# nicolapiccinelli/libmpc

Measured on AMD Instinct MI355X. Metric: MPC solves/sec (whole node) + p50 solve latency, quadrotor LMPC N=20 batch=4096, higher is better.
Workload: dtype f64; 1 GPU; quadrotor_ex.cpp LMPC nx=12 nu=4 ny=12 ph=ch=20, batch 4096 per GPU, SplitMix64 x0/u0/yref (SURVEY 8d), maximum_iteration=250; parallelism=single GPU, rccl_ranks=0, streams=1

## Files before the change

### libmpc_amd/csrc/lmpc_fast.hip

```cpp
#include "lmpc_kernel_common.hpp"
#include <cstddef>
#include <cstdlib>
#include <utility>

namespace mpcx {

namespace {

#ifndef MPCX_FAST_PF_MAXCAP
#define MPCX_FAST_PF_MAXCAP 12
#endif
#ifndef MPCX_FAST_RB
#define MPCX_FAST_RB 4
#endif
#ifndef MPCX_FAST_PF
#define MPCX_FAST_PF 4
#endif
#ifndef MPCX_FAST_PF_ALL
#define MPCX_FAST_PF_ALL 6
#endif
#ifndef MPCX_FAST_NBUF
#define MPCX_FAST_NBUF 3
#endif
#ifndef MPCX_FAST_RB_DEEP
#define MPCX_FAST_RB_DEEP 2
#endif
#ifndef MPCX_FAST_DEEP_CHUNKS
#define MPCX_FAST_DEEP_CHUNKS 4
#endif
#ifndef MPCX_FAST_XBAR_CLASSES
#define MPCX_FAST_XBAR_CLASSES 0
#endif
#ifndef MPCX_FAST_LDSMULT_CLASSES
#define MPCX_FAST_LDSMULT_CLASSES 0x30
#endif
#ifndef MPCX_FAST_XBAR_CHUNKS
#define MPCX_FAST_XBAR_CHUNKS 4
#endif
#ifndef MPCX_FAST_XBAR_CHUNK
#define MPCX_FAST_XBAR_CHUNK 0x333442400ull
#endif
constexpr int fast_xbar_chunk(int cap) { return (int)((MPCX_FAST_XBAR_CHUNK >> (4 * (cap / 2))) & 15) > 0 ? (int)((MPCX_FAST_XBAR_CHUNK >> (4 * (cap / 2))) & 15) : 1; }
constexpr bool fast_class_bit(unsigned mask, int cap, int chunks) { return chunks <= MPCX_FAST_XBAR_CHUNKS && ((mask >> (cap / 2)) & 1u) != 0; }
#ifndef MPCX_FAST_STAGE
#define MPCX_FAST_STAGE() __builtin_amdgcn_sched_barrier(0)
#endif
constexpr int kFastCap = 16;
#ifndef MPCX_FAST_ADD_THETA_LATE
#define MPCX_FAST_ADD_THETA_LATE 0.02
#endif
#ifndef MPCX_FAST_SAFE_AFTER
#define MPCX_FAST_SAFE_AFTER 12
#endif

template <int CTRL>
__device__ __forceinline__ double dpp_mov_d(double v)
{
    const int lo = __builtin_amdgcn_mov_dpp(__double2loint(v), CTRL, 0xF, 0xF, true);
    const int hi = __builtin_amdgcn_mov_dpp(__double2hiint(v), CTRL, 0xF, 0xF, true);
    return __hiloint2double(hi, lo);
}
__device__ __forceinline__ double wave_max_dpp(double v)
{
    v = fmax(v, dpp_mov_d<0xB1>(v));
    v = fmax(v, dpp_mov_d<0x4E>(v));
    v = fmax(v, dpp_mov_d<0x141>(v));
    v = fmax(v, dpp_mov_d<0x140>(v));
    v = fmax(v, dpp_mov_d<0x142>(v));
    v = fmax(v, dpp_mov_d<0x143>(v));
    return readlane_d(v, 63);
}

#ifdef MPCX_PROFILE_ROUNDS
#define MPCX_LAP(k) do { const long long now_ = (long long)__builtin_readcyclecounter(); pacc[k] += now_ - plast; plast = now_; } while (0)
#define MPCX_LAP_WAIT(k) do { __builtin_amdgcn_s_waitcnt(0); MPCX_LAP(k); } while (0)
#define MPCX_PROF_ARGS , long long (&pacc)[6], long long &plast
#define MPCX_PROF_PASS , pacc, plast
#else
#define MPCX_LAP(k) do {} while (0)
#define MPCX_LAP_WAIT(k) do {} while (0)
#define MPCX_PROF_ARGS
#define MPCX_PROF_PASS
#endif

template <int CAP, int NLO, int CPZ, int CPG, bool XB = false, bool XL = false>
__device__ __forceinline__ int ws_solve_reg(const gdp gY, const int ldy, const int ldz, const int na, const int lane_in,
                                            const int *wsidx, const double *wsb, const double *t0s, double *lam,
                                            const unsigned (&offz)[CPZ], const unsigned (&offg)[CPG],
                                            double (&wv)[2 * CPZ], double (&gw)[2 * CPG], double &lmax MPCX_PROF_ARGS)
{
    constexpr bool DEEP = CPZ + CPG <= MPCX_FAST_DEEP_CHUNKS;
    constexpr int PF = CAP > MPCX_FAST_PF_MAXCAP ? 0 : (CAP <= (DEEP ? MPCX_FAST_PF_ALL : MPCX_FAST_PF) ? CAP : MPCX_FAST_PF);
    int lane = lane_in;
    asm volatile("" : "+v"(lane));
    const bool real = lane < na;
    const int li = real ? lane : 0;
    const int qi = wsidx[li];
    int qc[CAP];
#pragma unroll
    for (int c = 0; c < CAP; ++c) qc[c] = __builtin_amdgcn_readfirstlane(wsidx[(c < NLO || c < na) ? c : 0]);
    double Sr[CAP];
    const unsigned rowoff = (unsigned)(qi * ldy) * 8u;
    const char MPCX_GAS *const gYb = reinterpret_cast<const char MPCX_GAS *>(gY);
    auto y_at = [&](unsigned off) { return *reinterpret_cast<gdp>(gYb + off); };
    auto row_ld2 = [&](int q, unsigned off) { return *reinterpret_cast<const d2 MPCX_GAS *>(gYb + (unsigned)(q * ldy) * 8u + off); };
#pragma unroll
    for (int c = 0; c < CAP; ++c) Sr[c] = y_at(rowoff + (unsigned)qc[c] * 8u);
    const double dg = y_at(rowoff + (unsigned)qi * 8u);
    d2 pz[PF > 0 ? PF : 1][CPZ], pg[PF > 0 ? PF : 1][CPG];
#pragma unroll
    for (int u = 0; u < PF; ++u) {
#pragma unroll
        for (int c = 0; c < CPZ; ++c) pz[u][c] = row_ld2(qc[u], offz[c]);
#pragma unroll
        for (int c = 0; c < CPG; ++c) pg[u][c] = row_ld2(qc[u], offg[c]);
    }
    double y = real ? t0s[qi < ldz ? qi : qi - ldz + 128 * CPZ] - wsb[li] : 0.0;
    MPCX_LAP_WAIT(1);
    if (!real) {
#pragma unroll
        for (int c = 0; c < CAP; ++c) Sr[c] = 0.0;
    }
#pragma unroll
    for (int c = NLO; c < CAP; ++c) if (c >= na) Sr[c] = lane == c ? 1.0 : 0.0;
    const double pthr = 1e-11 * (real ? dg : 1.0);
    double mydinv = 1.0;
    unsigned long long dep = 0ull;
    auto gj_step = [&]<int K>() {
        dep |= __ballot(!(Sr[K] > pthr)) & (1ull << K);
        const double rinv = pivot_rcp(readlane_d(Sr[K], K));
        if constexpr (XB) {
            constexpr int NE = CAP - K, XCH = fast_xbar_chunk(CAP), NC = (NE + XCH - 1) / XCH;
            double pv[2][XCH];
            auto request = [&](const int c) {
#pragma unroll
                for (int u = 0; u < XCH; ++u) {
                    const int j = K + 1 + c * XCH + u;
                    if (j <= CAP) pv[c & 1][u] = swizzle_bcast_d<K>(j < CAP ? Sr[j < CAP ? j : 0] : y);
                }
            };
            request(0);
            if (lane == K) mydinv = rinv;
            asm volatile("" : "+v"(mydinv));
            const double m = Sr[K] * rinv;
#pragma unroll
            for (int c = 0; c < NC; ++c) {
                if (c + 1 < NC) request(c + 1);
                if (lane != K) {
#pragma unroll
                    for (int u = 0; u < XCH; ++u) {
                        const int j = K + 1 + c * XCH + u;
                        if (j < CAP) Sr[j] = fma(-m, pv[c & 1][u], Sr[j]);
                        else if (j == CAP) y = fma(-m, pv[c & 1][u], y);
                    }
                }
            }
        } else {
            double pj[CAP];
#pragma unroll
            for (int j = K + 1; j < CAP; ++j) pj[j] = readlane_d(Sr[j], K);
            const double py = readlane_d(y, K);
            if (lane == K) mydinv = rinv;
            else {
                const double m = Sr[K] * rinv;
#pragma unroll
                for (int j = K + 1; j < CAP; ++j) Sr[j] = fma(-m, pj[j], Sr[j]);
                y = fma(-m, py, y);
            }
        }
    };
    [&]<int... Ks>(std::integer_sequence<int, Ks...>) { (gj_step.template operator()<Ks>(), ...); }(std::make_integer_sequence<int, CAP>{});
    MPCX_LAP(2);
    if (dep != 0ull) return (int)__builtin_ctzll(dep);
    y *= mydinv;
    if (XL ? lane < CAP : real) lam[lane] = y;
    auto lam_pair = [&](const int a, double (&l2)[2]) {
        const double2 v = *reinterpret_cast<const double2 *>(lam + a);
        l2[0] = v.x; l2[1] = v.y;
    };
    constexpr int NLP = XL && PF > 0 ? PF / 2 : 1;
    double lamp[NLP][2];
    if constexpr (XL) {
        static_assert(CAP % 2 == 0 && PF % 2 == 0 && kFastCap % 2 == 0, "multipliers are read back in pairs");
        wave_sync();
#pragma unroll
        for (int p = 0; p < PF / 2; ++p) lam_pair(2 * p, lamp[p]);
    }
#pragma unroll
    for (int c = 0; c < CPZ; ++c) {
        const double2 v = *reinterpret_cast<const double2 *>(t0s + 128 * c + 2 * lane);
        wv[2 * c] = v.x; wv[2 * c + 1] = v.y;
    }
#pragma unroll
    for (int c = 0; c < CPG; ++c) {
        const double2 v = *reinterpret_cast<const double2 *>(t0s + 128 * CPZ + 128 * c + 2 * lane);
        gw[2 * c] = v.x; gw[2 * c + 1] = v.y;
// ... 211 lines not shown
    }
    const int solver_status = infeasible ? -3 : (fixed_violation ? -2 : 1);

    double w[NZS], f[NZS];
    const double qnan = __builtin_nan("");
#pragma unroll
    for (int c = 0; c < CPZ; ++c) {
        const double2 vf = *reinterpret_cast<const double2 *>(fs + 128 * c + 2 * lane);
        f[2 * c] = vf.x; f[2 * c + 1] = vf.y;
    }
#pragma unroll
    for (int s = 0; s < NZS; ++s) w[s] = infeasible ? qnan : ((128 * (s >> 1) + 2 * lane + (s & 1) < nz) ? wv[s] : 0.0);
    double *stage = fs;
    double cost;
    bool cost_pending = false;
    wave_sync();
#pragma unroll
    for (int c = 0; c < CPZ; ++c) *reinterpret_cast<double2 *>(stage + 128 * c + 2 * lane) = make_double2(w[2 * c], w[2 * c + 1]);
    wave_sync();
    if (infeasible) {
        cost = 1e30;
    } else if (!M.cost_direct) {
        double j = 0;
#pragma unroll
        for (int s = 0; s < NZS; ++s) j = fma(f[s], w[s], j);
        if (lane < na_last) j = fma(-lam[lane], wsb[lane], j);
        cost = 0.5 * wave_sum(j) + c0;
    } else if (!FUSED && Bt.n_models <= 0) {
#pragma unroll
        for (int c = 0; c < CPZ; ++c) {
            const int e = 128 * c + 2 * lane;
            if (e < ldz) st2(ws + ldz + e, w[2 * c], w[2 * c + 1]);
        }
        cost = 0.0;
        cost_pending = true;
    } else {
        double hw[NZS];
#pragma unroll
        for (int s = 0; s < NZS; ++s) hw[s] = 0;
        matvec_acc<CPZ>(GP(H), ldz, ldz, nz, stage, hw, lane);
        double j = 0;
#pragma unroll
        for (int s = 0; s < NZS; ++s) j += w[s] * (0.5 * hw[s] + f[s]);
        cost = wave_sum(j) + c0;
    }
#pragma unroll
    for (int s = 0; s < NZS; ++s) {
        const int e = 128 * (s >> 1) + 2 * lane + (s & 1);
        if (e < nu) { if (outs) outs[8 + e] = w[s]; else glw(Bt.cmd)[(size_t)b * nu + e] = w[s]; }
    }
    if (outs) {
        if (lane == 0) {
            outs[0] = cost; outs[1] = solver_status == 1 ? 0 : (solver_status == -2 ? 1 : 2); outs[2] = solver_status;
            outs[3] = solver_status == -3 ? 0 : 1; outs[4] = 0; outs[5] = rounds_total; outs[6] = infeasible ? 0 : na_last; outs[7] = 2.0;
        }
    } else if (lane == 0) {
        if (Bt.cost && !cost_pending) glw(Bt.cost)[b] = cost;
        if (Bt.solver_status) glw(Bt.solver_status)[b] = solver_status;
        if (Bt.status) glw(Bt.status)[b] = solver_status == 1 ? 0 : (solver_status == -2 ? 1 : 2);
        if (Bt.is_feasible) glw(Bt.is_feasible)[b] = solver_status == -3 ? 0 : 1;
        if (Bt.iterations) glw(Bt.iterations)[b] = 0;
        if (Bt.polish_rounds) glw(Bt.polish_rounds)[b] = rounds_total;
        if (Bt.active_count) glw(Bt.active_count)[b] = infeasible ? 0 : na_last;
    }

    if (Bt.active_lower && Bt.active_upper) {
        wave_sync();
        unsigned *bl = reinterpret_cast<unsigned *>(t0s);
        unsigned *bu = bl + M.active_words;
        for (int wd = lane; wd < 2 * M.active_words; wd += 64) bl[wd] = 0u;
        wave_sync();
        if (!infeasible) {
#pragma unroll
            for (int s = 0; s < NZS; ++s) {
                const int e = 128 * (s >> 1) + 2 * lane + (s & 1);
                if (e >= nz || actb[s] == 0) continue;
                const double l = lam[posb[s]];
                if (!(fabs(l) > dtol_last)) continue;
                const int side = l < 0 ? -1 : 1;
                const double lo = lws[e], hi = uws[e];
                for (int p = GP(boxrow_ptr)[e]; p < GP(boxrow_ptr)[e + 1]; ++p) {
                    const int rr = GP(boxrow_ref)[p];
                    if (side < 0 && GP(boxrow_lo)[p] == lo) atomicOr(&bl[rr >> 5], 1u << (rr & 31));
                    if (side > 0 && GP(boxrow_hi)[p] == hi) atomicOr(&bu[rr >> 5], 1u << (rr & 31));
                }
            }
#pragma unroll
            for (int s = 0; s < NGS; ++s) {
                const int r = 128 * (s >> 1) + 2 * lane + (s & 1);
                if (r >= mg || actg[s] == 0) continue;
                const double l = lam[posg[s]];
                if (!(fabs(l) > dtol_last)) continue;
                const int rr = GP(g_refrow)[r];
                if (l < 0) atomicOr(&bl[rr >> 5], 1u << (rr & 31));
                else atomicOr(&bu[rr >> 5], 1u << (rr & 31));
            }
        }
        wave_sync();
        for (int wd = lane; wd < M.active_words; wd += 64) {
            glw(Bt.active_lower)[(size_t)b * M.active_words + wd] = bl[wd];
            glw(Bt.active_upper)[(size_t)b * M.active_words + wd] = bu[wd];
        }
        wave_sync();
    }

    if (Bt.seq_state || Bt.seq_input || Bt.seq_output) {
        wave_sync();
        const gdp gA = GP(A), gB = GP(B), gC = GP(C), gBd = GP(Bd), gDd = GP(Dd), gdm = gl(Bt.dmeas ? Bt.dmeas : M.dmeas_s);
        const gip gblk = GP(blk);
        auto dm = [&](int k, int dd) -> double { return ref_at(gdm, Bt.dmeas_bs, Bt.dmeas_ks, b, k, dd); };
        double *xs0 = scratch, *xs1 = scratch + nx;
        if (lane < nx) xs0[lane] = infeasible ? qnan : gl(Bt.x0)[(size_t)b * nx + lane];
        wave_sync();
        for (int i = 0; i <= ph; ++i) {
            const double *xc = (i & 1) ? xs1 : xs0;
            double *xn = (i & 1) ? xs0 : xs1;
            const int k = i > 0 ? i - 1 : 0;
            if (Bt.seq_state && lane < nx) glw(Bt.seq_state)[((size_t)b * (ph + 1) + i) * nx + lane] = xc[lane];
            if (Bt.seq_input && lane < nu) {
                const int ii = (i + 1 <= ph) ? i + 1 : ph;
                glw(Bt.seq_input)[((size_t)b * (ph + 1) + i) * nu + lane] = stage[gblk[ii] * nu + lane];
            }
            if (Bt.seq_output && lane < ny) {
                double yv = 0;
                for (int c = 0; c < nx; ++c) yv = fma(gC[lane + c * ny], xc[c], yv);
                if (M.has_dist) for (int dd = 0; dd < ndu; ++dd) yv = fma(gDd[lane + dd * ny], dm(k, dd), yv);
                glw(Bt.seq_output)[((size_t)b * (ph + 1) + i) * ny + lane] = yv;
            }
            if (i < ph && lane < nx) {
                double s = 0;
                for (int c = 0; c < nx; ++c) s = fma(gA[lane + c * nx], xc[c], s);
                for (int c = 0; c < nu; ++c) s = fma(gB[lane + c * nx], stage[gblk[i + 1] * nu + c], s);
                if (M.has_dist) for (int dd = 0; dd < ndu; ++dd) s = fma(gBd[lane + dd * nx], dm(i, dd), s);
                xn[lane] = s;
            }
            wave_sync();
        }
    }
    wave_sync();
    if (lane == 0 && !outs) ws[ldz + ldy + 2 * ldg + 1] = cost_pending ? 3.0 : 2.0;
    stamp(ts3);
    if (Bt.dbg_cycles && lane == 0)
    {
        long long *o = Bt.dbg_cycles + (size_t)b * 8;
#ifdef MPCX_PROFILE_ROUNDS
        o[0] = ts1 - ts0; o[1] = ts2 - ts1;
        for (int k = 0; k < 6; ++k) o[2 + k] = pacc[k];
#else
        o[0] = ts0; o[1] = ts1; o[2] = ts2; o[3] = ts3;
#endif
    }
}

template <int CPZ, int CPG, int SRC = 0>
__device__ __forceinline__ void solve_fast(const LmpcDev &M, const LmpcBatchDev &Bt, const int b, const int lane,
                           double *slice, const double *lwuw, gdw ws, const double *mf_lds = nullptr, double *outs = nullptr, const int eqbits = 0)
{
    constexpr int NZS = 2 * CPZ, NGS = 2 * CPG, ZP = 128 * CPZ, GPD = 128 * CPG;
    const int nz = M.nz, mg = M.mg, ldz = M.ldz, ldg = M.ldg, ldy = M.ldy;
    const gdp gY = GP(Y);
    double *t0s = slice, *gt0s = t0s + ZP, *lgs = gt0s + GPD, *ugs = lgs + GPD, *fs = ugs + GPD, *tail = fs + ZP;
    double *lam = tail + 2, *wsb = lam + (kFastCap + 2);
    int *wsidx = reinterpret_cast<int *>(wsb + (kFastCap + 2));
    double *scratch = wsb + (kFastCap + 2) + (kFastCap + 2) / 2 + 1;
    const double *lws = lwuw, *uws = lwuw + ZP;
    const double INF = __builtin_huge_val();

    long long ts0 = 0, ts1 = 0, ts2 = 0;
#ifdef MPCX_PROFILE_ROUNDS
    long long pacc[6] = {0, 0, 0, 0, 0, 0}, plast = 0;
#endif
    auto stamp = [&](long long &t) { if (Bt.dbg_cycles) t = (long long)__builtin_readcyclecounter(); };
    stamp(ts0);

    int offz[CPZ], offg[CPG];
#pragma unroll
    for (int c = 0; c < CPZ; ++c) { const int e = 128 * c + 2 * lane; offz[c] = e < ldz ? e : 0; }
#pragma unroll
    for (int c = 0; c < CPG; ++c) { const int r = 128 * c + 2 * lane; offg[c] = ldz + (r < ldg ? r : 0); }
    unsigned boffz[CPZ], boffg[CPG];
#pragma unroll
    for (int c = 0; c < CPZ; ++c) boffz[c] = (unsigned)offz[c] * 8u;
#pragma unroll
    for (int c = 0; c < CPG; ++c) boffg[c] = (unsigned)offg[c] * 8u;

    if constexpr (SRC != 2) fast_init_pads<CPZ, CPG>(slice, ldz, ldg, lane);
    if constexpr (SRC == 2) {
    } else if constexpr (SRC == 1) {
        RecPtrs rp{fs, t0s, gt0s, lgs, ugs, tail};
        fused_record(M, Bt, b, lane, scratch, rp, mf_lds);
    } else {
#pragma unroll
        for (int c = 0; c < CPZ; ++c) {
            const int e = 128 * c + 2 * lane;
            if (e < ldz) {
                const d2 vf = ld2(ws + e), vt = ld2(ws + ldz + e);
                *reinterpret_cast<double2 *>(fs + e) = make_double2(vf.x, vf.y);
                *reinterpret_cast<double2 *>(t0s + e) = make_double2(vt.x, vt.y);
            }
        }
#pragma unroll
        for (int c = 0; c < CPG; ++c) {
            const int r = 128 * c + 2 * lane;
            if (r < ldg) {
                const d2 vt = ld2(ws + 2 * ldz + r), vl = ld2(ws + ldz + ldy + r), vu = ld2(ws + ldz + ldy + ldg + r);
                *reinterpret_cast<double2 *>(gt0s + r) = make_double2(vt.x, vt.y);
                *reinterpret_cast<double2 *>(lgs + r) = make_double2(vl.x, vl.y);
                *reinterpret_cast<double2 *>(ugs + r) = make_double2(vu.x, vu.y);
            }
        }
        if (lane == 0) { const d2 t = ld2(ws + ldz + ldy + 2 * ldg); *reinterpret_cast<double2 *>(tail) = make_double2(t.x, t.y); }
        wave_sync();
    }
    const double flag0 = tail[1];
    const bool fixed_violation = flag0 == 1.0;
    const bool infeasible = fixed_violation && M.strict_infeasible;

    int actb[NZS], actg[NGS];
    const double ptol = 1e-8;
    auto viol = [&](double v, double lo, double hi) {
        const double lo_wide = fma(-ptol, fmax(1.0, fabs(lo)), lo), hi_scale = fmax(1.0, fabs(hi));
        return fmax(fmax(lo_wide - v, fma(-ptol, hi_scale, v - hi)), 0.0);
    };
    auto wrong_signed = [](double lm, int act) {
        const int in = -(act & 1);
        const int hi = (__double2hiint(lm) ^ (int)((unsigned)(act + 1) << 30)) & in;
        return __hiloint2double(hi, __double2loint(lm) & in);
    };
    {
        double vb[NZS], vg[NGS], vinit = 0.0;
        bool lowb[NZS], lowg[NGS];
#pragma unroll
        for (int c = 0; c < CPZ; ++c) {
            const int e = 128 * c + 2 * lane;
            const double2 l = *reinterpret_cast<const double2 *>(lws + e), u = *reinterpret_cast<const double2 *>(uws + e);
            const double2 t = *reinterpret_cast<const double2 *>(t0s + e);
            vb[2 * c] = viol(t.x, l.x, u.x); vb[2 * c + 1] = viol(t.y, l.y, u.y);
            lowb[2 * c] = t.x < l.x; lowb[2 * c + 1] = t.y < l.y;
            actb[2 * c] = l.x == u.x ? 2 : 0; actb[2 * c + 1] = l.y == u.y ? 2 : 0;
            vinit = fmax(vinit, fmax(vb[2 * c], vb[2 * c + 1]));
        }
#pragma unroll
        for (int c = 0; c < CPG; ++c) {
            const int r = 128 * c + 2 * lane;
            const double2 l = *reinterpret_cast<const double2 *>(lgs + r), u = *reinterpret_cast<const double2 *>(ugs + r);
            const double2 t = *reinterpret_cast<const double2 *>(gt0s + r);
            vg[2 * c] = viol(t.x, l.x, u.x); vg[2 * c + 1] = viol(t.y, l.y, u.y);
            lowg[2 * c] = t.x < l.x; lowg[2 * c + 1] = t.y < l.y;
            if constexpr (SRC == 2) {
                actg[2 * c] = ((eqbits >> (2 * c)) & 1) ? 2 : 0; actg[2 * c + 1] = ((eqbits >> (2 * c + 1)) & 1) ? 2 : 0;
            } else {
                const d2 l0 = ld2(GP(lg0) + (offg[c] - ldz)), u0 = ld2(GP(ug0) + (offg[c] - ldz));
                const bool ok = r < ldg;
                actg[2 * c] = (ok && l0.x == u0.x) ? 2 : 0; actg[2 * c + 1] = (ok && l0.y == u0.y) ? 2 : 0;
            }
            vinit = fmax(vinit, fmax(vg[2 * c], vg[2 * c + 1]));
        }
        const double thr0 = MPCX_INIT_THETA * wave_max_dpp(vinit);
#pragma unroll
        for (int s = 0; s < NZS; ++s) actb[s] = (actb[s] == 0 && vb[s] > 0.0 && vb[s] >= thr0) ? (lowb[s] ? -1 : 1) : actb[s];
#pragma unroll
        for (int s = 0; s < NGS; ++s) actg[s] = (actg[s] == 0 && vg[s] > 0.0 && vg[s] >= thr0) ? (lowg[s] ? -1 : 1) : actg[s];
    }
    stamp(ts1);

    if (Bt.warm_lower) {
        const unsigned MPCX_GAS *wl = gl(Bt.warm_lower) + (size_t)b * M.active_words;
        const unsigned MPCX_GAS *wu = gl(Bt.warm_upper) + (size_t)b * M.active_words;
        const int na = M.nx + M.nu, n1 = M.ph + 1;
        const int b_box = M.neq_ref, b_out = b_box + n1 * na, b_du = b_out + n1 * M.ny, b_sc = b_du + M.ph * M.nu;
        auto look = [&](int rr) {
            if (!Bt.warm_shift) return rr;
            if (rr < b_out) return rr + na < b_out ? rr + na : rr;
            if (rr < b_du) return rr + M.ny < b_du ? rr + M.ny : rr;
            if (rr < b_sc) return rr;
            return rr + 1 < M.m_ref ? rr + 1 : rr;
        };
#pragma unroll
        for (int s = 0; s < NZS; ++s) {
            const int e = 128 * (s >> 1) + 2 * lane + (s & 1);
            if (e >= nz || actb[s] == 2) continue;
            const double lo = lws[e], hi = uws[e];
            int side = 0;
            for (int p = GP(boxrow_ptr)[e]; p < GP(boxrow_ptr)[e + 1]; ++p) {
                const int rr = look(GP(boxrow_ref)[p]);
                if (((wl[rr >> 5] >> (rr & 31)) & 1u) && GP(boxrow_lo)[p] == lo) side = -1;
                if (((wu[rr >> 5] >> (rr & 31)) & 1u) && GP(boxrow_hi)[p] == hi) side = 1;
            }
            actb[s] = side;
        }
#pragma unroll
        for (int s = 0; s < NGS; ++s) {
            const int r = 128 * (s >> 1) + 2 * lane + (s & 1);
            if (r >= mg || actg[s] == 2) continue;
            const int rr = look(GP(g_refrow)[r]);
            actg[s] = ((wl[rr >> 5] >> (rr & 31)) & 1u) ? -1 : (((wu[rr >> 5] >> (rr & 31)) & 1u) ? 1 : 0);
        }
    }

    double wv[NZS], gw[NGS];
    int posb[NZS], posg[NGS];
    double dtol_last = 0;
    int na_last = 0, rounds_total = 0;
    bool solved = false;

    if (!infeasible && M.polish) {
        const int rounds = M.polish_rounds0;
        for (int rd = 0; rd < rounds; ++rd) {
            ++rounds_total;
#ifdef MPCX_PROFILE_ROUNDS
            plast = (long long)__builtin_readcyclecounter();
#endif
            if (rd == 3) __builtin_amdgcn_s_setprio(1);
            else if (rd == 5) __builtin_amdgcn_s_setprio(2);
            else if (rd == 7) __builtin_amdgcn_s_setprio(3);
            int na = 0;
#pragma unroll
            for (int c = 0; c < CPZ; ++c) {
                const int e = 128 * c + 2 * lane;
                const double2 l = *reinterpret_cast<const double2 *>(lws + e), u = *reinterpret_cast<const double2 *>(uws + e);
#pragma unroll
                for (int h = 0; h < 2; ++h) {
                    const int s = 2 * c + h;
                    const bool act = actb[s] != 0;
                    const unsigned long long mk = __ballot(act);
                    int pos = (int)__builtin_amdgcn_mbcnt_hi((unsigned)(mk >> 32), __builtin_amdgcn_mbcnt_lo((unsigned)mk, (unsigned)na));
                    pos = (act && pos < kFastCap) ? pos : kFastCap;
                    posb[s] = pos;
                    wsidx[pos] = e + h;
                    wsb[pos] = actb[s] < 0 ? (h ? l.y : l.x) : (h ? u.y : u.x);
                    na += __popcll(mk);
                }
            }
#pragma unroll
            for (int c = 0; c < CPG; ++c) {
                const int r = 128 * c + 2 * lane;
                const double2 l = *reinterpret_cast<const double2 *>(lgs + r), u = *reinterpret_cast<const double2 *>(ugs + r);
#pragma unroll
                for (int h = 0; h < 2; ++h) {
                    const int s = 2 * c + h;
                    const bool act = actg[s] != 0;
                    const unsigned long long mk = __ballot(act);
                    int pos = (int)__builtin_amdgcn_mbcnt_hi((unsigned)(mk >> 32), __builtin_amdgcn_mbcnt_lo((unsigned)mk, (unsigned)na));
                    pos = (act && pos < kFastCap) ? pos : kFastCap;
                    posg[s] = pos;
                    wsidx[pos] = ldz + r + h;
                    wsb[pos] = actg[s] < 0 ? (h ? l.y : l.x) : (h ? u.y : u.x);
                    na += __popcll(mk);
                }
            }
            if (na > kFastCap) break;
            na_last = na;
            wave_sync();
            MPCX_LAP_WAIT(0);
            int dep_at = -1;
            double lmax = 0.0;
            constexpr auto xb = [](int cap) { return SRC != 1 && fast_class_bit(MPCX_FAST_XBAR_CLASSES, cap, CPZ + CPG); };
            constexpr auto xl = [](int cap) { return SRC != 1 && fast_class_bit(MPCX_FAST_LDSMULT_CLASSES, cap, CPZ + CPG); };
            if (na == 0) {
#pragma unroll
                for (int c = 0; c < CPZ; ++c) { const double2 v = *reinterpret_cast<const double2 *>(t0s + 128 * c + 2 * lane); wv[2 * c] = v.x; wv[2 * c + 1] = v.y; }
#pragma unroll
                for (int c = 0; c < CPG; ++c) { const double2 v = *reinterpret_cast<const double2 *>(gt0s + 128 * c + 2 * lane); gw[2 * c] = v.x; gw[2 * c + 1] = v.y; }
            } else if (na <= 4) dep_at = ws_solve_reg<4, 1, CPZ, CPG, xb(4), xl(4)>(gY, ldy, ldz, na, lane, wsidx, wsb, t0s, lam, boffz, boffg, wv, gw, lmax MPCX_PROF_PASS);
            else if (na <= 6) dep_at = ws_solve_reg<6, 5, CPZ, CPG, xb(6), xl(6)>(gY, ldy, ldz, na, lane, wsidx, wsb, t0s, lam, boffz, boffg, wv, gw, lmax MPCX_PROF_PASS);
            else if (na <= 8) dep_at = ws_solve_reg<8, 7, CPZ, CPG, xb(8), xl(8)>(gY, ldy, ldz, na, lane, wsidx, wsb, t0s, lam, boffz, boffg, wv, gw, lmax MPCX_PROF_PASS);
            else if (na <= 10) dep_at = ws_solve_reg<10, 9, CPZ, CPG, xb(10), xl(10)>(gY, ldy, ldz, na, lane, wsidx, wsb, t0s, lam, boffz, boffg, wv, gw, lmax MPCX_PROF_PASS);
            else if (na <= 12) dep_at = ws_solve_reg<12, 11, CPZ, CPG, xb(12), xl(12)>(gY, ldy, ldz, na, lane, wsidx, wsb, t0s, lam, boffz, boffg, wv, gw, lmax MPCX_PROF_PASS);
            else if (na <= 14) dep_at = ws_solve_reg<14, 13, CPZ, CPG, xb(14), xl(14)>(gY, ldy, ldz, na, lane, wsidx, wsb, t0s, lam, boffz, boffg, wv, gw, lmax MPCX_PROF_PASS);
            else dep_at = ws_solve_reg<kFastCap, 15, CPZ, CPG, xb(kFastCap), xl(kFastCap)>(gY, ldy, ldz, na, lane, wsidx, wsb, t0s, lam, boffz, boffg, wv, gw, lmax MPCX_PROF_PASS);
            if (dep_at >= 0) {
                const int q = wsidx[dep_at];
#pragma unroll
                for (int s = 0; s < NZS; ++s)
                    if (128 * (s >> 1) + 2 * lane + (s & 1) == q) actb[s] = 0;
#pragma unroll
                for (int s = 0; s < NGS; ++s)
                    if (ldz + 128 * (s >> 1) + 2 * lane + (s & 1) == q) actg[s] = 0;
                wave_sync();
                continue;
            }
            wave_sync();
            MPCX_LAP_WAIT(3);
            const double dtol = 1e-9 * lmax + 1e-300;
            dtol_last = dtol;
            double badb[NZS], badg[NGS], vb[NZS], vg[NGS], vm = 0.0, bm = 0.0, chk = 0.0;
            bool lowb[NZS], lowg[NGS];
            double lmb[NZS], lmg[NGS];
#pragma unroll
            for (int s = 0; s < NZS; ++s) lmb[s] = lam[posb[s]];
#pragma unroll
            for (int s = 0; s < NGS; ++s) lmg[s] = lam[posg[s]];
#pragma unroll
            for (int c = 0; c < CPZ; ++c) {
                const int e = 128 * c + 2 * lane;
                const double2 l = *reinterpret_cast<const double2 *>(lws + e), u = *reinterpret_cast<const double2 *>(uws + e);
#pragma unroll
                for (int h = 0; h < 2; ++h) {
                    const int s = 2 * c + h;
                    const double lo = h ? l.y : l.x, hi = h ? u.y : u.x;
                    chk += wv[s];
                    lowb[s] = wv[s] < lo;
                    const double v = viol(wv[s], lo, hi);
                    vb[s] = actb[s] == 0 ? v : 0.0;
                    badb[s] = wrong_signed(lmb[s], actb[s]);
                    vm = fmax(vm, vb[s]); bm = fmax(bm, badb[s]);
                }
            }
#pragma unroll
            for (int c = 0; c < CPG; ++c) {
                const int r = 128 * c + 2 * lane;
                const double2 l = *reinterpret_cast<const double2 *>(lgs + r), u = *reinterpret_cast<const double2 *>(ugs + r);
#pragma unroll
                for (int h = 0; h < 2; ++h) {
                    const int s = 2 * c + h;
                    const double lo = h ? l.y : l.x, hi = h ? u.y : u.x;
                    chk += gw[s];
                    lowg[s] = gw[s] < lo;
                    const double v = viol(gw[s], lo, hi);
                    vg[s] = actg[s] == 0 ? v : 0.0;
                    badg[s] = wrong_signed(lmg[s], actg[s]);
                    vm = fmax(vm, vg[s]); bm = fmax(bm, badg[s]);
                }
            }
            if (wave_any(!(chk - chk == 0.0))) break;
            MPCX_LAP(4);
            const bool any_bad = wave_any(bm > dtol), any_viol = wave_any(vm > 0.0);
            if (!any_bad && !any_viol) { solved = true; break; }
            if (rd < MPCX_FAST_SAFE_AFTER) {
                const double thr = any_viol ? (rd < 3 ? MPCX_FAST_ADD_THETA : MPCX_FAST_ADD_THETA_LATE) * wave_max_dpp(vm) : INF;
#pragma unroll
                for (int s = 0; s < NZS; ++s) actb[s] = badb[s] > dtol ? 0 : ((vb[s] > 0.0 && vb[s] >= thr) ? (lowb[s] ? -1 : 1) : actb[s]);
#pragma unroll
                for (int s = 0; s < NGS; ++s) actg[s] = badg[s] > dtol ? 0 : ((vg[s] > 0.0 && vg[s] >= thr) ? (lowg[s] ? -1 : 1) : actg[s]);
            } else {
                const double mx = wave_max_dpp(any_bad ? bm : vm);
                int slot = -1;
#pragma unroll
                for (int s = 0; s < NZS; ++s) if (slot < 0 && (any_bad ? badb[s] : vb[s]) == mx) slot = s;
#pragma unroll
                for (int s = 0; s < NGS; ++s) if (slot < 0 && (any_bad ? badg[s] : vg[s]) == mx) slot = NZS + s;
                const unsigned long long mk = __ballot(slot >= 0);
                if (slot >= 0 && lane == (int)__builtin_ctzll(mk)) {
#pragma unroll
                    for (int s = 0; s < NZS; ++s) if (slot == s) actb[s] = any_bad ? 0 : (lowb[s] ? -1 : 1);
#pragma unroll
                    for (int s = 0; s < NGS; ++s) if (slot == NZS + s) actg[s] = any_bad ? 0 : (lowg[s] ? -1 : 1);
                }
            }
            wave_sync();
            MPCX_LAP(5);
        }
    }
    __builtin_amdgcn_s_setprio(0);
    stamp(ts2);

    if constexpr (SRC == 2) {
        group_args_p ka = (group_args_p)__builtin_amdgcn_kernarg_segment_ptr();
        asm volatile("" : "+s"(ka));
        fast_finish<CPZ, CPG, SRC>((const LmpcDev &)ka->M, (const LmpcBatchDev &)ka->Bt, b, lane, slice, lwuw, ws, outs, infeasible, solved, fixed_violation,
                                   wv, actb, actg, posb, posg, dtol_last, na_last, rounds_total, ts0, ts1, ts2 MPCX_PROF_PASS);
    } else {
        fast_finish<CPZ, CPG, SRC>(M, Bt, b, lane, slice, lwuw, ws, outs, infeasible, solved, fixed_violation,
                                   wv, actb, actg, posb, posg, dtol_last, na_last, rounds_total, ts0, ts1, ts2 MPCX_PROF_PASS);
    }
}

#ifndef MPCX_FAST_WAVES1
#define MPCX_FAST_WAVES1 4
#endif
#ifndef MPCX_FAST_WAVES2
#define MPCX_FAST_WAVES2 2
#endif
template <int CPZ> constexpr int fast_waves() { return CPZ == 1 ? MPCX_FAST_WAVES1 : (CPZ == 2 ? MPCX_FAST_WAVES2 : 2); }

template <int CPZ>
__device__ __forceinline__ void fast_load_box(const LmpcDev &M, double *lwuw)
{
    constexpr int ZP = 128 * CPZ;
    const double INF = __builtin_huge_val();
    for (int e = 2 * (int)threadIdx.x; e < ZP; e += 2 * (int)blockDim.x) {
        const bool ok = e < M.ldz;
        const d2 vl = ld2(GP(lw) + (ok ? e : 0)), vu = ld2(GP(uw) + (ok ? e : 0));
        *reinterpret_cast<double2 *>(lwuw + e) = ok ? make_double2(vl.x, vl.y) : make_double2(-INF, -INF);
        *reinterpret_cast<double2 *>(lwuw + ZP + e) = ok ? make_double2(vu.x, vu.y) : make_double2(INF, INF);
    }
    __syncthreads();
}

template <int CPZ, int CPG>
__global__ __launch_bounds__(kWavesPerBlock * 64, fast_waves<CPZ>()) void lmpc_solve(const LmpcDev *__restrict__ Mp, const LmpcBatchDev Bt, double *wsbase)
{
    extern __shared__ __attribute__((aligned(16))) double smem[];
    const LmpcDev &M = *Mp;
    const int lane = threadIdx.x & 63, wave = __builtin_amdgcn_readfirstlane(threadIdx.x >> 6);
    constexpr int ZP = 128 * CPZ;
    const int wpb = blockDim.x >> 6;
    double *rec = smem + 2 * ZP + (size_t)wave * M.fast_slice;
    fast_load_box<CPZ>(M, smem);
    const int i = blockIdx.x * wpb + wave;
    if (i < Bt.batch) solve_fast<CPZ, CPG, 0>(M, Bt, i, lane, rec, smem, glw(wsbase) + (size_t)i * M.wsld);
}

template <int CPZ, int CPG>
__global__ __launch_bounds__(kWavesPerBlock * 64, fast_waves<CPZ>()) void lmpc_solve_hetero(const LmpcDev *__restrict__ Mp, const LmpcBatchDev Bt, double *wsbase)
{
    extern __shared__ __attribute__((aligned(16))) double smem[];
    const LmpcDev &M = *Mp;
    const int lane = threadIdx.x & 63, wave = __builtin_amdgcn_readfirstlane(threadIdx.x >> 6);
    constexpr int ZP = 128 * CPZ;
    const int wpb = blockDim.x >> 6;
    double *rec = smem + 2 * ZP + (size_t)wave * M.fast_slice;
    double *box = smem + 2 * ZP + (size_t)wpb * M.fast_slice + (size_t)wave * 2 * ZP;
    const double INF = __builtin_huge_val();
    const int i = blockIdx.x * wpb + wave;
    if (i < Bt.batch) {
        const LmpcDev &Mi = Mp[lmpc_model_of(Bt, i)];
#pragma unroll
        for (int c = 0; c < CPZ; ++c) {
            const int e = 128 * c + 2 * lane;
            const bool ok = e < Mi.ldz;
            const d2 vl = ld2(gl(Mi.lw) + (ok ? e : 0)), vu = ld2(gl(Mi.uw) + (ok ? e : 0));
            *reinterpret_cast<double2 *>(box + e) = ok ? make_double2(vl.x, vl.y) : make_double2(-INF, -INF);
            *reinterpret_cast<double2 *>(box + ZP + e) = ok ? make_double2(vu.x, vu.y) : make_double2(INF, INF);
        }
        wave_sync();
        solve_fast<CPZ, CPG, 0>(Mi, Bt, i, lane, rec, box, glw(wsbase) + (size_t)i * M.wsld);
        wave_sync();
    }
}

template <int CPZ, int CPG>
__global__ __launch_bounds__(kWavesPerBlock * 64, fast_waves<CPZ>()) void lmpc_solve_fused(const LmpcDev *__restrict__ Mp, const LmpcBatchDev Bt, double *wsbase)
{
    extern __shared__ __attribute__((aligned(16))) double smem[];
    const LmpcDev &M = *Mp;
    const int lane = threadIdx.x & 63, wave = __builtin_amdgcn_readfirstlane(threadIdx.x >> 6);
    fast_load_box<CPZ>(M, smem);
    double *rec = smem + 2 * 128 * CPZ + (size_t)wave * M.fast_slice;
    const int wpb = blockDim.x >> 6;
    const int b = blockIdx.x * wpb + wave;
    if (b < Bt.batch) solve_fast<CPZ, CPG, 1>(M, Bt, b, lane, rec, smem, glw(wsbase) + (size_t)b * M.wsld);
}

constexpr int kPersistWaves = 12;
template <int CPZ, int CPG>
__global__ __launch_bounds__(kPersistWaves * 64) void lmpc_solve_persistent(const LmpcDev *__restrict__ Mp, const LmpcBatchDev Bt, double *wsbase,
                                                                             int *counter)
{
    extern __shared__ __attribute__((aligned(16))) double smem[];
    const LmpcDev &M = *Mp;
    const int lane = threadIdx.x & 63, wave = __builtin_amdgcn_readfirstlane(threadIdx.x >> 6);
    const int nmf = M.rowsF * M.kin;
    {
        const gdp src = gl(Bt.fused == 2 ? M.MF1 : M.MF0);
        for (int k = 2 * (int)threadIdx.x; k < nmf; k += 2 * (int)blockDim.x) {
            const d2 v = ld2(src + k);
            *reinterpret_cast<double2 *>(smem + k) = make_double2(v.x, v.y);
        }
    }
    double *lwuw = smem + nmf;
    fast_load_box<CPZ>(M, lwuw);
    double *rec = lwuw + 2 * 128 * CPZ + (size_t)wave * M.fast_slice;
    const int nwaves = gridDim.x * kPersistWaves, shard = blockIdx.x & 7;
    int b = blockIdx.x * kPersistWaves + wave;
    while (b < Bt.batch) {
        solve_fast<CPZ, CPG, 1>(M, Bt, b, lane, rec, lwuw, glw(wsbase) + (size_t)b * M.wsld, smem);
        int n = 0;
        if (lane == 0) n = atomicAdd(counter + shard, 1);
        n = __builtin_amdgcn_readfirstlane(n);
        b = nwaves + shard + 8 * n;
    }
}

template <size_t BYTES>
__device__ __forceinline__ void kernarg_touch()
{
    static_assert(BYTES <= 16 * 64 && BYTES > 15 * 64, "kernarg_touch covers sixteen lines, the sixteenth must exist");
    const auto ka = __builtin_amdgcn_kernarg_segment_ptr();
    int t0, t1, t2, t3, t4, t5, t6, t7, t8, t9, t10, t11, t12, t13, t14, t15;
    asm volatile("s_load_dword %0, %16, 0x0\n\ts_load_dword %1, %16, 0x40\n\ts_load_dword %2, %16, 0x80\n\ts_load_dword %3, %16, 0xc0\n\t"
                 "s_load_dword %4, %16, 0x100\n\ts_load_dword %5, %16, 0x140\n\ts_load_dword %6, %16, 0x180\n\ts_load_dword %7, %16, 0x1c0\n\t"
                 "s_load_dword %8, %16, 0x200\n\ts_load_dword %9, %16, 0x240\n\ts_load_dword %10, %16, 0x280\n\ts_load_dword %11, %16, 0x2c0\n\t"
                 "s_load_dword %12, %16, 0x300\n\ts_load_dword %13, %16, 0x340\n\ts_load_dword %14, %16, 0x380\n\ts_load_dword %15, %16, 0x3c0\n\t"
                 "s_waitcnt lgkmcnt(0)"
                 : "=&s"(t0), "=&s"(t1), "=&s"(t2), "=&s"(t3), "=&s"(t4), "=&s"(t5), "=&s"(t6), "=&s"(t7), "=&s"(t8), "=&s"(t9), "=&s"(t10), "=&s"(t11),
                   "=&s"(t12), "=&s"(t13), "=&s"(t14), "=&s"(t15)
                 : "s"(ka)
                 : "memory");
}
#ifndef MPCX_GROUP_BALANCE
#define MPCX_GROUP_BALANCE 1
#endif

template <int CPZ> constexpr int kGroupWavesOf = CPZ == 1 ? 16 : 8;
constexpr int kGroupG2 = 5;
constexpr int kGroupG1 = 2;
template <int CPZ, int CPG>
__global__ __launch_bounds__(kGroupWavesOf<CPZ> * 64) void lmpc_solve_group(const LmpcDev Mv, const LmpcBatchDev Btv, double *wsbasev, const int variantv)
{
    constexpr int kGroupWaves = kGroupWavesOf<CPZ>;
    extern __shared__ __attribute__((aligned(16))) double smem[];
#if defined(MPCX_GROUP_CUT) && MPCX_GROUP_CUT == 0
// ... 363 lines not shown
```

Before: 126.1 million solves/s.

## Build next working set at end of round and add exact-size small solve classes

```diff
diff --git a/libmpc_amd/csrc/lmpc_fast.hip b/libmpc_amd/csrc/lmpc_fast.hip
--- a/libmpc_amd/csrc/lmpc_fast.hip
+++ b/libmpc_amd/csrc/lmpc_fast.hip
@@ -40,8 +40,14 @@
 #ifndef MPCX_FAST_XBAR_CHUNK
 #define MPCX_FAST_XBAR_CHUNK 0x333442400ull
 #endif
-constexpr int fast_xbar_chunk(int cap) { return (int)((MPCX_FAST_XBAR_CHUNK >> (4 * (cap / 2))) & 15) > 0 ? (int)((MPCX_FAST_XBAR_CHUNK >> (4 * (cap / 2))) & 15) : 1; }
-constexpr bool fast_class_bit(unsigned mask, int cap, int chunks) { return chunks <= MPCX_FAST_XBAR_CHUNKS && ((mask >> (cap / 2)) & 1u) != 0; }
+constexpr int fast_xbar_chunk(int cap) { return (int)((MPCX_FAST_XBAR_CHUNK >> (4 * ((cap + 1) / 2))) & 15) > 0 ? (int)((MPCX_FAST_XBAR_CHUNK >> (4 * ((cap + 1) / 2))) & 15) : 1; }
+constexpr bool fast_class_bit(unsigned mask, int cap, int chunks) { return cap % 2 == 0 && chunks <= MPCX_FAST_XBAR_CHUNKS && ((mask >> (cap / 2)) & 1u) != 0; }
+#ifndef MPCX_FAST_EXACT_CLASSES
+#define MPCX_FAST_EXACT_CLASSES 0x2Eu
+#endif
+#ifndef MPCX_FAST_BUILD_BEHIND
+#define MPCX_FAST_BUILD_BEHIND 1
+#endif
 #ifndef MPCX_FAST_STAGE
 #define MPCX_FAST_STAGE() __builtin_amdgcn_sched_barrier(0)
 #endif
@@ -559,7 +565,9 @@
     }
 }
 
-template <int CPZ, int CPG, int SRC = 0>
+template <int CPZ, int CPG> constexpr unsigned fast_exact_classes() { return CPZ + CPG == 4 ? MPCX_FAST_EXACT_CLASSES : 0u; }
+template <int CPZ, int CPG> constexpr bool fast_build_behind() { return MPCX_FAST_BUILD_BEHIND != 0 && CPZ + CPG == 4; }
+template <int CPZ, int CPG, int SRC = 0, unsigned EXACT = fast_exact_classes<CPZ, CPG>(), bool BEHIND = fast_build_behind<CPZ, CPG>()>
 __device__ __forceinline__ void solve_fast(const LmpcDev &M, const LmpcBatchDev &Bt, const int b, const int lane,
                            double *slice, const double *lwuw, gdw ws, const double *mf_lds = nullptr, double *outs = nullptr, const int eqbits = 0)
 {
@@ -713,19 +721,12 @@
 
     if (!infeasible && M.polish) {
         const int rounds = M.polish_rounds0;
-        for (int rd = 0; rd < rounds; ++rd) {
-            ++rounds_total;
-#ifdef MPCX_PROFILE_ROUNDS
-            plast = (long long)__builtin_readcyclecounter();
-#endif
-            if (rd == 3) __builtin_amdgcn_s_setprio(1);
-            else if (rd == 5) __builtin_amdgcn_s_setprio(2);
-            else if (rd == 7) __builtin_amdgcn_s_setprio(3);
+        auto build_set = [&]<bool REGS>(const double2 (&lz)[CPZ], const double2 (&uz)[CPZ], const double2 (&lgv)[CPG], const double2 (&ugv)[CPG]) {
             int na = 0;
 #pragma unroll
             for (int c = 0; c < CPZ; ++c) {
                 const int e = 128 * c + 2 * lane;
-                const double2 l = *reinterpret_cast<const double2 *>(lws + e), u = *reinterpret_cast<const double2 *>(uws + e);
+                const double2 l = REGS ? lz[c] : *reinterpret_cast<const double2 *>(lws + e), u = REGS ? uz[c] : *reinterpret_cast<const double2 *>(uws + e);
 #pragma unroll
                 for (int h = 0; h < 2; ++h) {
                     const int s = 2 * c + h;
@@ -742,7 +743,7 @@
 #pragma unroll
             for (int c = 0; c < CPG; ++c) {
                 const int r = 128 * c + 2 * lane;
-                const double2 l = *reinterpret_cast<const double2 *>(lgs + r), u = *reinterpret_cast<const double2 *>(ugs + r);
+                const double2 l = REGS ? lgv[c] : *reinterpret_cast<const double2 *>(lgs + r), u = REGS ? ugv[c] : *reinterpret_cast<const double2 *>(ugs + r);
 #pragma unroll
                 for (int h = 0; h < 2; ++h) {
                     const int s = 2 * c + h;
@@ -756,6 +757,24 @@
                     na += __popcll(mk);
                 }
             }
+            return na;
+        };
+        auto build_set_lds = [&]() {
+            const double2 nz[CPZ] = {}, ng[CPG] = {};
+            return build_set.template operator()<false>(nz, nz, ng, ng);
+        };
+        int na_next = 0;
+        if constexpr (BEHIND) na_next = build_set_lds();
+        for (int rd = 0; rd < rounds; ++rd) {
+            ++rounds_total;
+#ifdef MPCX_PROFILE_ROUNDS
+            plast = (long long)__builtin_readcyclecounter();
+#endif
+            if (rd == 3) __builtin_amdgcn_s_setprio(1);
+            else if (rd == 5) __builtin_amdgcn_s_setprio(2);
+            else if (rd == 7) __builtin_amdgcn_s_setprio(3);
+            int na = na_next;
+            if constexpr (!BEHIND) na = build_set_lds();
             if (na > kFastCap) break;
             na_last = na;
             wave_sync();
@@ -764,13 +783,21 @@
             double lmax = 0.0;
             constexpr auto xb = [](int cap) { return SRC != 1 && fast_class_bit(MPCX_FAST_XBAR_CLASSES, cap, CPZ + CPG); };
             constexpr auto xl = [](int cap) { return SRC != 1 && fast_class_bit(MPCX_FAST_LDSMULT_CLASSES, cap, CPZ + CPG); };
+            constexpr auto ex = [](int cap) { return ((EXACT >> cap) & 1u) != 0; };
+            constexpr int NLO4 = !ex(1) ? 1 : (!ex(2) ? 2 : (!ex(3) ? 3 : 4)), NLO6 = ex(5) ? 6 : 5;
+#define MPCX_WS_CLASS(CAP_, NLO_) ws_solve_reg<CAP_, NLO_, CPZ, CPG, xb(CAP_), xl(CAP_)>(gY, ldy, ldz, na, lane, wsidx, wsb, t0s, lam, boffz, boffg, wv, gw, lmax MPCX_PROF_PASS)
             if (na == 0) {
 #pragma unroll
                 for (int c = 0; c < CPZ; ++c) { const double2 v = *reinterpret_cast<const double2 *>(t0s + 128 * c + 2 * lane); wv[2 * c] = v.x; wv[2 * c + 1] = v.y; }
 #pragma unroll
                 for (int c = 0; c < CPG; ++c) { const double2 v = *reinterpret_cast<const double2 *>(gt0s + 128 * c + 2 * lane); gw[2 * c] = v.x; gw[2 * c + 1] = v.y; }
-            } else if (na <= 4) dep_at = ws_solve_reg<4, 1, CPZ, CPG, xb(4), xl(4)>(gY, ldy, ldz, na, lane, wsidx, wsb, t0s, lam, boffz, boffg, wv, gw, lmax MPCX_PROF_PASS);
-            else if (na <= 6) dep_at = ws_solve_reg<6, 5, CPZ, CPG, xb(6), xl(6)>(gY, ldy, ldz, na, lane, wsidx, wsb, t0s, lam, boffz, boffg, wv, gw, lmax MPCX_PROF_PASS);
+            } else if (ex(1) && na == 1) dep_at = MPCX_WS_CLASS(1, 1);
+            else if (ex(2) && na == 2) dep_at = MPCX_WS_CLASS(2, 2);
+            else if (ex(3) && na == 3) dep_at = MPCX_WS_CLASS(3, 3);
+            else if (na <= 4) dep_at = MPCX_WS_CLASS(4, NLO4);
+            else if (ex(5) && na == 5) dep_at = MPCX_WS_CLASS(5, 5);
+            else if (na <= 6) dep_at = MPCX_WS_CLASS(6, NLO6);
+#undef MPCX_WS_CLASS
             else if (na <= 8) dep_at = ws_solve_reg<8, 7, CPZ, CPG, xb(8), xl(8)>(gY, ldy, ldz, na, lane, wsidx, wsb, t0s, lam, boffz, boffg, wv, gw, lmax MPCX_PROF_PASS);
             else if (na <= 10) dep_at = ws_solve_reg<10, 9, CPZ, CPG, xb(10), xl(10)>(gY, ldy, ldz, na, lane, wsidx, wsb, t0s, lam, boffz, boffg, wv, gw, lmax MPCX_PROF_PASS);
             else if (na <= 12) dep_at = ws_solve_reg<12, 11, CPZ, CPG, xb(12), xl(12)>(gY, ldy, ldz, na, lane, wsidx, wsb, t0s, lam, boffz, boffg, wv, gw, lmax MPCX_PROF_PASS);
@@ -785,6 +812,7 @@
                 for (int s = 0; s < NGS; ++s)
                     if (ldz + 128 * (s >> 1) + 2 * lane + (s & 1) == q) actg[s] = 0;
                 wave_sync();
+                if constexpr (BEHIND) na_next = build_set_lds();
                 continue;
             }
             wave_sync();
@@ -794,6 +822,7 @@
             double badb[NZS], badg[NGS], vb[NZS], vg[NGS], vm = 0.0, bm = 0.0, chk = 0.0;
             bool lowb[NZS], lowg[NGS];
             double lmb[NZS], lmg[NGS];
+            double2 lz[CPZ], uz[CPZ], lgv[CPG], ugv[CPG];
 #pragma unroll
             for (int s = 0; s < NZS; ++s) lmb[s] = lam[posb[s]];
 #pragma unroll
@@ -802,6 +831,7 @@
             for (int c = 0; c < CPZ; ++c) {
                 const int e = 128 * c + 2 * lane;
                 const double2 l = *reinterpret_cast<const double2 *>(lws + e), u = *reinterpret_cast<const double2 *>(uws + e);
+                lz[c] = l; uz[c] = u;
 #pragma unroll
                 for (int h = 0; h < 2; ++h) {
                     const int s = 2 * c + h;
@@ -818,6 +848,7 @@
             for (int c = 0; c < CPG; ++c) {
                 const int r = 128 * c + 2 * lane;
                 const double2 l = *reinterpret_cast<const double2 *>(lgs + r), u = *reinterpret_cast<const double2 *>(ugs + r);
+                lgv[c] = l; ugv[c] = u;
 #pragma unroll
                 for (int h = 0; h < 2; ++h) {
                     const int s = 2 * c + h;
@@ -840,6 +871,7 @@
                 for (int s = 0; s < NZS; ++s) actb[s] = badb[s] > dtol ? 0 : ((vb[s] > 0.0 && vb[s] >= thr) ? (lowb[s] ? -1 : 1) : actb[s]);
 #pragma unroll
                 for (int s = 0; s < NGS; ++s) actg[s] = badg[s] > dtol ? 0 : ((vg[s] > 0.0 && vg[s] >= thr) ? (lowg[s] ? -1 : 1) : actg[s]);
+                if constexpr (BEHIND) na_next = build_set.template operator()<true>(lz, uz, lgv, ugv);
             } else {
                 const double mx = wave_max_dpp(any_bad ? bm : vm);
                 int slot = -1;
@@ -854,8 +886,9 @@
 #pragma unroll
                     for (int s = 0; s < NGS; ++s) if (slot == NZS + s) actg[s] = any_bad ? 0 : (lowg[s] ? -1 : 1);
                 }
-            }
-            wave_sync();
+                if constexpr (BEHIND) { wave_sync(); na_next = build_set_lds(); }
+            }
+            if constexpr (!BEHIND) wave_sync();
             MPCX_LAP(5);
         }
     }
```

Result: no change. 126.2 million solves/s (median of 3 runs) (+0.1%).
